# TruongKhang/cds-mvsnet

Hardware: AMD Instinct MI355X
Metric: depth-maps/sec per ref view at 640x512 N=5 D=192 (single-stage plane sweep incl. CostRegNet + regression) (higher is better)
Workload: dtype f32; 1 GPU; M1: single-stage StageNet volume 640x512, D=192, C=8, N=5 views; parallelism=single

## Files before the change

### cds_mvsnet_amd/csrc/cds_common.hpp

```cpp
#pragma once
#include <hip/hip_runtime.h>
#include <stdint.h>
#include <stdlib.h>

#include <atomic>

#include "../../include/cds_mvsnet_hip.h"

#define CDS_WAVE 64

#define CDS_ZMG_UNSUPPORTED 1
int cds_conv3d_zmg_dispatch(const float* x, const void* wsp, const float* bias, float* out, int Cin, int Cout, int D, int H, int W,
                            int stride, int pair, int act, hipStream_t st, const float* in_bound = nullptr, float w_inv = 1.f,
                            float* out_bound = nullptr);

using cds_f4 = float __attribute__((ext_vector_type(4)));

extern "C" int cds_debug_poison_lds(unsigned pattern);

static inline int cds_launch_status() {
  hipError_t e = hipGetLastError();
  if (const char* p = getenv("CDS_DEBUG_POISON_LDS")) {
    if (e == hipSuccess) (void)cds_debug_poison_lds((unsigned)strtoul(p, nullptr, 16));
  }
  return e == hipSuccess ? 0 : -(int)e;
}

static inline int cds_ceil_div(int a, int b) { return (a + b - 1) / b; }

static inline bool cds_env_is(const char* name, char c) { const char* e = getenv(name); return e && e[0] == c; }
static inline bool cds_env_set(const char* name) { return getenv(name) != nullptr; }
static inline int cds_env_int(const char* name, int dflt) { const char* e = getenv(name); return e ? atoi(e) : dflt; }

static inline int cds_allow_lds(const void* kernel, int bytes, std::atomic<unsigned long long>& mask) {
  int d = 0;
  (void)hipGetDevice(&d);
  const unsigned long long bit = 1ull << (d & 63);
  if (mask.load(std::memory_order_acquire) & bit) return 0;
  hipError_t e = hipFuncSetAttribute(kernel, hipFuncAttributeMaxDynamicSharedMemorySize, bytes);
  if (e != hipSuccess) { (void)hipGetLastError(); return -(int)e; }
  mask.fetch_or(bit, std::memory_order_release);
  return 0;
}

__device__ __forceinline__ int cds_xcd_remap(int bid, int nwg) {
  const int nx = 8;
  if (nwg < 2 * nx) return bid;
  int q = nwg / nx, r = nwg % nx;
  int xcd = bid % nx, idx = bid / nx;
  int base = xcd < r ? xcd * (q + 1) : r * (q + 1) + (xcd - r) * q;
  return base + idx;
}

__device__ __forceinline__ const float* cds_uniform_ptr(const float* p) {
  const uint64_t u = reinterpret_cast<uint64_t>(p);
  const uint32_t lo = __builtin_amdgcn_readfirstlane((uint32_t)u);
  const uint32_t hi = __builtin_amdgcn_readfirstlane((uint32_t)(u >> 32));
  return reinterpret_cast<const float*>(((uint64_t)hi << 32) | lo);
}

__device__ __forceinline__ float cds_act_conv(float v, int act) {
  if (act == CDS_ACT_RELU) return fmaxf(v, 0.0f);
  if (act == CDS_ACT_SIGMOID) return 1.0f / (1.0f + expf(-v));
  return v;
}

__device__ __forceinline__ float cds_apply_act(float v, int act) {
  switch (act) {
    case CDS_ACT_RELU: return fmaxf(v, 0.0f);
    case CDS_ACT_LEAKY01: return v > 0.0f ? v : v * 0.1f;
    case CDS_ACT_SIGMOID: return 1.0f / (1.0f + expf(-v));
    case CDS_ACT_TANH: return tanhf(v);
    default: return v;
  }
}
```

### cds_mvsnet_amd/csrc/conv3d_sbf.hip

```cpp
#include <stdlib.h>

#include "cds_common.hpp"
#include "sbf_common.hpp"

namespace {

#ifdef CDS_SBF_XFAST
#define SBF_TILE(tile, A, B, C) const int A = (tile) % tiles_x, B = ((tile) / tiles_x) % tiles_y, C = (tile) / (tiles_x * tiles_y)
#else
#define SBF_TILE(tile, A, B, C) \
  const int tiles_z_ = ntiles / (tiles_x * tiles_y); \
  const int C = (tile) % tiles_z_, A = ((tile) / tiles_z_) % tiles_x, B = (tile) / (tiles_z_ * tiles_x)
#endif

template <int S, int MB, int TX_, int TZ_, bool PAIR = false, bool WRES_ = false>
struct FCfg {
  static constexpr int TX = TX_, TY = 4, TZ = TZ_;
  static constexpr bool DEINT = S == 2 || PAIR;
  static constexpr int XT = TX / (PAIR ? 32 : 16), NT = XT * TZ;
  static constexpr int IX = (TX - 1) * S + 3, IY = (TY - 1) * S + 3, IZ = (TZ - 1) * S + 3;
  static constexpr int IXH = DEINT ? (IX + 1) / 2 : 0;
  static constexpr int IXP = DEINT ? 2 * IXH : (IX + 7) / 8 * 8;
  static constexpr int NPOS = IZ * IY * IXP;
  static constexpr int LDSB = NPOS * POSB;
// ... 698 lines not shown
      const unsigned char* tbuf = tiles + (st & 1) * Cfg::LDSB;
      const unsigned char* wr = wlds + rd * Tab::NKS * 3 * 1024;
      BV wa[2][3];
      BV bd[2][Cfg::NT][3];
      auto load_w = [&](int buf, int ks) {
        wa[buf][0].u = *reinterpret_cast<const uint4*>(wr + (ks * 3) * 1024);
        wa[buf][1].u = *reinterpret_cast<const uint4*>(wr + (ks * 3 + 1) * 1024);
        wa[buf][2].u = *reinterpret_cast<const uint4*>(wr + (ks * 3 + 2) * 1024);
      };
      auto load_b = [&](int buf, int ks) {
        const unsigned char* bp = tbuf + b_base + toff[ks];
#pragma unroll
        for (int q = 0; q < Cfg::NT; ++q) {
          const unsigned char* b = bp + q * 16 * POSB;
          bd[buf][q][0].u = *reinterpret_cast<const uint4*>(b);
          bd[buf][q][1].u = *reinterpret_cast<const uint4*>(b + 16);
          bd[buf][q][2].u = *reinterpret_cast<const uint4*>(b + 32);
        }
      };
      load_w(0, 0);
      load_b(0, 0);
#pragma unroll
      for (int ks = 0; ks < Tab::NKS; ++ks) {
        const int c = Tab::cls_of(ks), cur = ks & 1;
        if (ks + 1 < Tab::NKS) {
          load_b(cur ^ 1, ks + 1);
          load_w(cur ^ 1, ks + 1);
        }
        __builtin_amdgcn_sched_barrier(0);
        SBF_TERMS(acc[c], 0, Cfg::NT, wa[cur], bd[cur]);
      }
      if (rd + 1 == rounds && ay < H) {
#pragma unroll
        for (int c = 0; c < Tab::NCLS; ++c) {
          const size_t rowbase = ((size_t)(2 * az + (c >> 1)) * Ho + (2 * ay + (c & 1))) * Wo;
#pragma unroll
          for (int q = 0; q < Cfg::NT; ++q) {
            const int ax = tx_i * Cfg::CX + q * 16 + j;
            if (ax >= W) continue;
            const size_t base = (rowbase + 2 * ax + px) * Cout + co;
            const f32x4 a = acc[c][q];
            float4 o = make_float4(a.x + bv.x, a.y + bv.y, a.z + bv.z, a.w + bv.w);
            if (act == CDS_ACT_RELU) {
              o.x = fmaxf(o.x, 0.f); o.y = fmaxf(o.y, 0.f); o.z = fmaxf(o.z, 0.f); o.w = fmaxf(o.w, 0.f);
            }
            if (skip) {
              const float4 s4 = skv[c][q];
              o.x = s4.x + o.x; o.y = s4.y + o.y; o.z = s4.z + o.z; o.w = s4.w + o.w;
            }
            if (out_planar) {
              const size_t ovol = (size_t)(2 * D) * Ho * Wo;
              float* po = out + (size_t)co * ovol + (rowbase + 2 * ax + px);
#ifdef CDS_SBF_NTSTORE
              __builtin_nontemporal_store(o.x, po); __builtin_nontemporal_store(o.y, po + ovol);
              __builtin_nontemporal_store(o.z, po + 2 * ovol); __builtin_nontemporal_store(o.w, po + 3 * ovol);
#else
              po[0] = o.x; po[ovol] = o.y; po[2 * ovol] = o.z; po[3 * ovol] = o.w;
#endif
            } else {
              sbf_store4(out + base, o);
            }
          }
        }
      }
      __syncthreads();
    }
  }
}

template <int CYT>
int launch_deconv_ws_t(const float* x, const void* wsp, const float* b, const float* skip, float* out, int Cin, int Cout, int D, int H,
                       int W, int act, int out_planar, hipStream_t st) {
  using Cfg = DWSCfg<CYT>;
  const int tx = cds_ceil_div(W, Cfg::CX), ty = cds_ceil_div(H, Cfg::CY);
  const int ntiles = tx * ty * D;
  int tpw = max(1, min(16, ntiles / (256 * (CYT == 8 ? 1 : 2) * 8)));
  const int nwg = cds_ceil_div(ntiles, tpw);
  const int lds_bytes = (Cin >> 3) * DTab<true>::NKS * 3 * 1024 + 2 * Cfg::LDSB;
  static std::atomic<unsigned long long> lds_ok{0};
  if (int e_lds = cds_allow_lds(reinterpret_cast<const void*>(deconv3d_sbf_ws_kernel<CYT>), 160 * 1024, lds_ok)) return e_lds;
  hipLaunchKernelGGL(deconv3d_sbf_ws_kernel<CYT>, dim3(nwg), dim3(Cfg::THREADS), lds_bytes, st, x, reinterpret_cast<const uint4*>(wsp), b,
                     skip, out, Cin, Cout, D, H, W, act, out_planar, tx, ty, ntiles, tpw);
  return cds_launch_status();
}

int launch_deconv_ws(const float* x, const void* wsp, const float* b, const float* skip, float* out, int Cin, int Cout, int D, int H,
                     int W, int act, int out_planar, hipStream_t st) {
  const bool big = (H >= 16 && (long)cds_ceil_div(W, 32) * cds_ceil_div(H, 8) * D >= 2 * 256);
  if (big) return launch_deconv_ws_t<8>(x, wsp, b, skip, out, Cin, Cout, D, H, W, act, out_planar, st);
  return launch_deconv_ws_t<4>(x, wsp, b, skip, out, Cin, Cout, D, H, W, act, out_planar, st);
}

}

extern "C" int cds_conv3d_sbf_f32(const float* x, const void* weight_split, const float* bias, const float* skip, float* out,
                                  int Cin, int Cout, int D, int H, int W, int stride, int act, void* stream) {
  if (!x || !weight_split || !out || Cin < 8 || (Cin % 8) || Cout < 4 || (Cout % 4) || Cout > 64 || D < 1 || H < 1 || W < 1 ||
      (stride != 1 && stride != 2 && stride != CDS_SBF_PAIR))
    return CDS_EINVAL;
  if (stride == CDS_SBF_PAIR && Cout != 8) return CDS_EINVAL;
  hipStream_t st = (hipStream_t)stream;
  const int mb = (Cout + 15) / 16;
  if (!skip) {
    const int r = cds_conv3d_zmg_dispatch(x, weight_split, bias, out, Cin, Cout, D, H, W, stride == CDS_SBF_PAIR ? 1 : stride,
                                          stride == CDS_SBF_PAIR, act, st);
    if (r != CDS_ZMG_UNSUPPORTED) return r;
  }
  if (stride == CDS_SBF_PAIR) {
    if (Cout != 8) return CDS_EINVAL;
    if (Cin == 8) return launch_fwd<1, 1, 32, 4, true, true>(x, weight_split, bias, skip, out, Cin, Cout, D, H, W, act, st);
    return launch_fwd<1, 1, 32, 4, true>(x, weight_split, bias, skip, out, Cin, Cout, D, H, W, act, st);
  }
  if (stride == 1) {
    if (mb == 1) return launch_fwd<1, 1, 32, 4>(x, weight_split, bias, skip, out, Cin, Cout, D, H, W, act, st);
    if (mb == 2) return launch_fwd<1, 2, 32, 2>(x, weight_split, bias, skip, out, Cin, Cout, D, H, W, act, st);
    if (mb == 4) return launch_fwd<1, 4, 32, 2>(x, weight_split, bias, skip, out, Cin, Cout, D, H, W, act, st);
    return CDS_EINVAL;
  }
  if (mb == 1) return launch_fwd<2, 1, 16, 2>(x, weight_split, bias, skip, out, Cin, Cout, D, H, W, act, st);
  if (mb == 2) return launch_fwd<2, 2, 16, 2>(x, weight_split, bias, skip, out, Cin, Cout, D, H, W, act, st);
  if (mb == 4) return launch_fwd<2, 4, 16, 2>(x, weight_split, bias, skip, out, Cin, Cout, D, H, W, act, st);
  return CDS_EINVAL;
}

extern "C" int cds_conv3d_sf16_f32(const float* x, const void* weight_split, const float* bias, float* out, int Cin, int Cout, int D, int H,
                                   int W, int stride, int act, const float* in_bound, float w_inv_scale, float* out_bound, void* stream) {
  if (!x || !weight_split || !out || !in_bound || Cin < 8 || (Cin % 8) || Cout < 4 || (Cout % 4) || Cout > 64 || D < 1 || H < 1 || W < 1 ||
      (stride != 1 && stride != 2 && stride != CDS_SBF_PAIR) || !(w_inv_scale > 0.f))
    return CDS_EINVAL;
  if (stride == CDS_SBF_PAIR && Cout != 8) return CDS_EINVAL;
  hipStream_t st = (hipStream_t)stream;
  const int r = cds_conv3d_zmg_dispatch(x, weight_split, bias, out, Cin, Cout, D, H, W, stride == CDS_SBF_PAIR ? 1 : stride,
                                        stride == CDS_SBF_PAIR, act, st, in_bound, w_inv_scale, out_bound);
  if (r != CDS_ZMG_UNSUPPORTED) return r;
  const int mb = (Cout + 15) / 16;
  const int s_ = stride, Do = (D - 1) / s_ + 1, Ho = (H - 1) / s_ + 1, Wo = (W - 1) / s_ + 1;
  const long tiles = (long)cds_ceil_div(Wo, s_ == 1 ? 32 : 16) * cds_ceil_div(Ho, 4) * cds_ceil_div(Do, 2);
  const bool split = tiles <= cds_env_int("CDS_SBF_YSPLIT_TILES", 256) && !cds_env_is("CDS_SBF_YSPLIT", '0');
  if (split && stride == 1 && (mb == 2 || mb == 4))
    return launch_fwd<1, 1, 32, 2, false, false, true>(x, weight_split, bias, nullptr, out, Cin, Cout, D, H, W, act, st, in_bound, w_inv_scale, out_bound, mb);
  if (split && stride == 2 && mb == 4)
    return launch_fwd<2, 1, 16, 2, false, false, true>(x, weight_split, bias, nullptr, out, Cin, Cout, D, H, W, act, st, in_bound, w_inv_scale, out_bound, mb);
  if (stride == 1 && mb == 2) return launch_fwd<1, 2, 32, 2, false, false, true>(x, weight_split, bias, nullptr, out, Cin, Cout, D, H, W, act, st, in_bound, w_inv_scale, out_bound);
  if (stride == 1 && mb == 4) return launch_fwd<1, 4, 32, 2, false, false, true>(x, weight_split, bias, nullptr, out, Cin, Cout, D, H, W, act, st, in_bound, w_inv_scale, out_bound);
  if (stride == 2 && mb == 4) return launch_fwd<2, 4, 16, 2, false, false, true>(x, weight_split, bias, nullptr, out, Cin, Cout, D, H, W, act, st, in_bound, w_inv_scale, out_bound);
  return CDS_EINVAL;
}

extern "C" int cds_deconv3d_sf16_f32(const float* x, const void* weight_split, const float* bias, const float* skip, float* out, int Cin,
                                     int Cout, int D, int H, int W, int act, const float* in_bound, float w_inv_scale, float* out_bound,
                                     void* stream) {
  if (!x || !weight_split || !out || !in_bound || Cin < 8 || (Cin % 8) || Cout != 32 || D < 1 || H < 1 || W < 1 || !(w_inv_scale > 0.f))
    return CDS_EINVAL;
  const long tiles = (long)cds_ceil_div(W, 32) * cds_ceil_div(H, 4) * D;
  if (tiles <= cds_env_int("CDS_SBF_YSPLIT_TILES", 256) && !cds_env_is("CDS_SBF_YSPLIT", '0'))
    return launch_deconv<false, 1, true>(x, weight_split, bias, skip, out, Cin, Cout, D, H, W, act, 0, (hipStream_t)stream, in_bound,
                                         w_inv_scale, out_bound, 2);
  return launch_deconv<false, 2, true>(x, weight_split, bias, skip, out, Cin, Cout, D, H, W, act, 0, (hipStream_t)stream, in_bound,
                                       w_inv_scale, out_bound);
}

extern "C" int cds_deconv3d_sbf_f32(const float* x, const void* weight_split, const float* bias, const float* skip, float* out,
                                    int Cin, int Cout, int D, int H, int W, int act, int out_planar, void* stream) {
  if (!x || !weight_split || !out || Cin < 8 || (Cin % 8) || D < 1 || H < 1 || W < 1) return CDS_EINVAL;
  hipStream_t st = (hipStream_t)stream;
  if (Cout == 8) {
    if (Cin <= 32) return launch_deconv_ws(x, weight_split, bias, skip, out, Cin, Cout, D, H, W, act, out_planar, st);
    return launch_deconv<true, 1>(x, weight_split, bias, skip, out, Cin, Cout, D, H, W, act, out_planar, st);
  }
  if (Cout == 16) return launch_deconv<false, 1>(x, weight_split, bias, skip, out, Cin, Cout, D, H, W, act, out_planar, st);
  if (Cout == 32) return launch_deconv<false, 2>(x, weight_split, bias, skip, out, Cin, Cout, D, H, W, act, out_planar, st);
  return CDS_EINVAL;
}
```

### cds_mvsnet_amd/csrc/conv3d_zmg.hip

```cpp
#include <stdlib.h>

#include "cds_common.hpp"
#include "sbf_common.hpp"

namespace {

__device__ __attribute__((aligned(32))) float g_zmg_zeros[8];

template <int S_, int RD_, int MB_, bool PAIR_, int TXO_, int TYO_, int G_, int NG_, int CW_ = 4, bool F16_ = false, int RPW_ = 1,
          int YS_ = 1, int PF_ = 1>
struct ZG {
  static constexpr int S = S_, RD = RD_, MB = MB_, TXO = TXO_, TYO = TYO_, G = G_, NG = NG_;
  static constexpr bool F16 = F16_;
  static constexpr int NT = F16_ ? 2 : 3;
  static constexpr bool PAIR = PAIR_, DEINT = PAIR_ || S_ == 2;
  static constexpr int CW = CW_, PW = 4, THREADS = (CW + PW) * 64;
  static constexpr int RPW = RPW_, YS = YS_, PF = PF_;
  static_assert(PF == 1 || (PF == 2 && 2 * NG_ * (F16_ ? 2 : 3) <= 15), "operand prefetch distance (lgkmcnt is a 4-bit count)");
  static_assert(RD % RPW == 0 && MB % YS == 0, "rounds per wave / cout split");
  static constexpr int KSPL = RD / RPW, MBS = MB / YS;
  static_assert(CW % (KSPL * MBS) == 0 && (KSPL == 1 || KSPL == 2 || KSPL == 4), "consumer waves");
  static constexpr int PARTS = CW / (KSPL * MBS);
  static constexpr int ROWS = TYO / PARTS;
  static constexpr int XT = TXO / (PAIR ? 32 : 16);
// ... 213 lines not shown
      for (int jf = 0; jf < Cfg::NFIN; ++jf) {
        const int n = jf * 4 + k;
        if (n >= NTW) continue;
        const unsigned char* src = xch + (sp & 1) * Cfg::XCH1 + ((xgrp + n) * 4) * 1024 + lane * 16;
        f32x4 total = KEEP4 && k == 0 ? keep[jf] : *reinterpret_cast<const f32x4*>(src);
#pragma unroll
        for (int kk = 1; kk < 4; ++kk) total = total + (KEEP4 && kk == k ? keep[jf] : *reinterpret_cast<const f32x4*>(src + kk * 1024));
        store_tile_rt(n, sp, total);
      }
    } else {
#pragma unroll
      for (int n = 0; n < NTW; ++n) store_tile(n, sp, acc[n]);
    }
  };
  __syncthreads();
  for (int st = 0; st < nstages; ++st) {
    if (late && st > 0) finish(st - 1);
    int vpl[PAIR ? Cfg::NRES : 1];
    int vaddr[PAIR ? 1 : KS][PAIR ? 1 : G];
    {
      int sl[Cfg::NRES];
      int slot = (st * S * G) % R;
#pragma unroll
      for (int u = 0; u < Cfg::NRES; ++u) {
        sl[u] = slot * Cfg::PLANEB;
        slot = slot + 1 >= R ? slot + 1 - R : slot + 1;
      }
      if (PAIR) {
#pragma unroll
        for (int u = 0; u < Cfg::NRES; ++u) vpl[u] = lane_base + sl[u];
      } else {
#pragma unroll
        for (int t = 0; t < KS; ++t)
#pragma unroll
          for (int i = 0; i < G; ++i) {
            const int o0 = sl[S * i + Cfg::tap_kz(t, 0)] + Cfg::tap_off(t, 0), o1 = sl[S * i + Cfg::tap_kz(t, 1)] + Cfg::tap_off(t, 1);
            const int o2 = sl[S * i + Cfg::tap_kz(t, 2)] + Cfg::tap_off(t, 2), o3 = sl[S * i + Cfg::tap_kz(t, 3)] + Cfg::tap_off(t, 3);
            vaddr[t][i] = lane_base + (g == 0 ? o0 : (g == 1 ? o1 : (g == 2 ? o2 : o3)));
          }
      }
    }
    constexpr int NGRP = NTW / NG, NS = RPW * KS * NGRP;
    constexpr int PF = Cfg::PF;
    BV bd[PF + 1][NG][NT];
    auto load_b = [&](int buf, int ss) {
      const int t = (ss / NGRP) % KS, rr = ss / (NGRP * KS), grp = ss % NGRP;
#pragma unroll
      for (int q = 0; q < NG; ++q) {
        const int n = grp * NG + q, i = n % G, rx = n / G, xt = rx % Cfg::XT, r = rx / Cfg::XT;
        const unsigned char* b = lds + (PAIR ? vpl[PAIR ? S * i + t / 3 : 0] + (t % 3) * Cfg::IXP * POSB : vaddr[PAIR ? 0 : t][PAIR ? 0 : i]) +
                                 (r * S * Cfg::IXP + xt * 16) * POSB + rr * Cfg::SLICEB;
        bd[buf][q][0].u = *reinterpret_cast<const uint4*>(b);
        bd[buf][q][1].u = *reinterpret_cast<const uint4*>(b + 16);
        if (!F16) bd[buf][q][NT - 1].u = *reinterpret_cast<const uint4*>(b + 32);
      }
    };
    load_b(0, 0);
    if (PF == 2 && NS > 1) load_b(1, 1);
    __builtin_amdgcn_s_setprio(0);
#pragma unroll
    for (int t = 0; t < NTW; ++t) acc[t] = (f32x4){0.f, 0.f, 0.f, 0.f};
#pragma unroll
    for (int ss = 0; ss < NS; ++ss) {
      const int t = ss / NGRP, grp = ss % NGRP, db = ss % (PF + 1);
      if (ss + PF < NS) load_b((ss + PF) % (PF + 1), ss + PF);
      __builtin_amdgcn_sched_barrier(0);
#ifndef CDS_ZMG_LAZYWAIT
      if (ss + PF < NS) __builtin_amdgcn_s_waitcnt(0xC07F | ((PF * NT * NG) << 8));
      else if (PF == 2 && ss + 1 < NS) __builtin_amdgcn_s_waitcnt(0xC07F | ((NT * NG) << 8));
      else __builtin_amdgcn_s_waitcnt(0xC07F);
      __builtin_amdgcn_sched_barrier(0);
#endif
      if constexpr (F16) {
        SF16_TERMS(acc, grp * NG, NG, wres[t], bd[db]);
      } else {
        SBF_TERMS(acc, grp * NG, NG, wres[t], bd[db]);
      }
    }
    __builtin_amdgcn_s_setprio(CDS_ZMG_CPRIO);
    if (Cfg::KSPL == 2) {
      if (!late && st > 0) finish(st - 1);
      unsigned char* dst = xch + (st & 1) * Cfg::XCH1 + (wave * NH) * 1024 + lane * 16;
#pragma unroll
      for (int m = 0; m < NH; ++m) {
        *reinterpret_cast<f32x4*>(dst + m * 1024) = acc[(k ^ 1) * NH + m];
        keep[m] = acc[k * NH + m];
      }
    } else if (Cfg::KSPL == 4) {
      if (!late && st > 0) finish(st - 1);
      unsigned char* dst = xch + (st & 1) * Cfg::XCH1 + (xgrp * 4 + k) * 1024 + lane * 16;
#pragma unroll
      for (int n = 0; n < NTW; ++n) {
        if (KEEP4 && (n & 3) == k) keep[n >> 2] = acc[n];
        else *reinterpret_cast<f32x4*>(dst + n * 4096) = acc[n];
      }
    } else if (!late) {
      finish(st);
    }
    __syncthreads();
  }
  if (Cfg::KSPL >= 2 || late) finish(nstages - 1);
  if (F16) sf16_publish_bound(amax, out_bound);
}

inline int zmg_pick_nseg(int cols, int Do, int G) {
  const int nseg_env = cds_env_int("CDS_ZMG_NSEG", 0);
  if (nseg_env > 0) return nseg_env;
  const int stages = cds_ceil_div(Do, G);
  int best = 1;
  double best_cost = 1e30;
  for (int n = 1; n <= 32 && n <= stages; ++n) {
    const int per = cds_ceil_div(stages, n);
    if (n > 1 && per < 6) break;
    const double cost = (double)cds_ceil_div(cols * cds_ceil_div(stages, per), 256) * (per + 2.5);
    if (cost < best_cost - 1e-9) { best_cost = cost; best = n; }
  }
  return best;
}

template <class Cfg>
int launch_zmg(const float* x, const void* wsp, const float* b, float* out, int Cout, int D, int H, int W, int act, hipStream_t st,
               const float* in_bound = nullptr, float w_inv = 1.f, float* out_bound = nullptr, int min_wgs = 0) {
  constexpr int S = Cfg::S;
  const int Do = (D - 1) / S + 1, Ho = (H - 1) / S + 1, Wo = (W - 1) / S + 1;
  const int tx = cds_ceil_div(Wo, Cfg::TXO), ty = cds_ceil_div(Ho, Cfg::TYO);
  int nseg = zmg_pick_nseg(tx * ty * Cfg::YS, Do, Cfg::G);
  const int zseg = cds_ceil_div(cds_ceil_div(Do, nseg), Cfg::G) * Cfg::G;
  nseg = cds_ceil_div(Do, zseg);
  if (min_wgs > 0 && tx * ty * nseg * Cfg::YS < min_wgs) return CDS_ZMG_UNSUPPORTED;
  auto kern = conv3d_zmg_kernel<Cfg>;
  static std::atomic<unsigned long long> lds_ok{0};
  if (int e_lds = cds_allow_lds(reinterpret_cast<const void*>(kern), Cfg::LDSB, lds_ok)) return e_lds;
  hipLaunchKernelGGL(kern, dim3(tx * ty * nseg, Cfg::YS), dim3(Cfg::THREADS), Cfg::LDSB, st, x, reinterpret_cast<const uint4*>(wsp), b,
                     out, Cout, D, H, W, Do, Ho, Wo, act, tx, ty, zseg, in_bound, w_inv, out_bound);
  return cds_launch_status();
}

}

int cds_conv3d_zmg_dispatch(const float* x, const void* wsp, const float* bias, float* out, int Cin, int Cout, int D, int H, int W,
                            int stride, int pair, int act, hipStream_t st, const float* in_bound, float w_inv, float* out_bound) {
  if (in_bound) {
    if (pair) {
      if (Cin == 8) return launch_zmg<ZG<1, 1, 1, true, 32, 8, 3, 1, 8, true>>(x, wsp, bias, out, Cout, D, H, W, act, st, in_bound, w_inv, out_bound);
      if (Cin == 16) return launch_zmg<ZG<1, 2, 1, true, 32, 8, 1, 4, 4, true>>(x, wsp, bias, out, Cout, D, H, W, act, st, in_bound, w_inv, out_bound);
      if (Cin == 32) return launch_zmg<ZG<1, 4, 1, true, 32, 3, 1, 3, 4, true>>(x, wsp, bias, out, Cout, D, H, W, act, st, in_bound, w_inv, out_bound);
      return CDS_ZMG_UNSUPPORTED;
    }
    if (stride == 1 && Cin == 16 && Cout == 16)
      return launch_zmg<ZG<1, 2, 1, false, 32, 8, 1, 1, 8, true>>(x, wsp, bias, out, Cout, D, H, W, act, st, in_bound, w_inv, out_bound);
    if (stride == 2 && Cin == 8 && Cout == 16)
      return launch_zmg<ZG<2, 1, 1, false, 16, 8, 1, 1, 8, true>>(x, wsp, bias, out, Cout, D, H, W, act, st, in_bound, w_inv, out_bound);
    if (stride == 2 && Cin == 16 && Cout == 32)
      return launch_zmg<ZG<2, 2, 2, false, 16, 4, 1, 1, 8, true>>(x, wsp, bias, out, Cout, D, H, W, act, st, in_bound, w_inv, out_bound);
    const int deep = cds_env_is("CDS_ZMG", '0') ? 0 : cds_env_int("CDS_ZMG_DEEP", 1);
    const int min_wgs = deep == 2 ? 0 : 256;
    if (deep > 0 && stride == 1 && Cin == 32 && Cout == 32)
      return launch_zmg<ZG<1, 4, 2, false, 16, 4, 1, 1, 8, true, 1, 1, 2>>(x, wsp, bias, out, Cout, D, H, W, act, st, in_bound, w_inv, out_bound, min_wgs);
    if (deep > 0 && stride == 1 && Cin == 64 && Cout == 64)
      return launch_zmg<ZG<1, 8, 4, false, 16, 2, 1, 1, 8, true, 2, 2>>(x, wsp, bias, out, Cout, D, H, W, act, st, in_bound, w_inv, out_bound, min_wgs);
    return CDS_ZMG_UNSUPPORTED;
  }
  const bool off = cds_env_is("CDS_ZMG", '0');
  if (off) return CDS_ZMG_UNSUPPORTED;
  if (pair) {
    if (Cin == 8) return launch_zmg<ZG<1, 1, 1, true, 32, 8, 3, 1, 8>>(x, wsp, bias, out, Cout, D, H, W, act, st);
    if (Cin == 16) return launch_zmg<ZG<1, 2, 1, true, 32, 8, 1, 4>>(x, wsp, bias, out, Cout, D, H, W, act, st);
    if (Cin == 32) return launch_zmg<ZG<1, 4, 1, true, 32, 3, 1, 3>>(x, wsp, bias, out, Cout, D, H, W, act, st);
    return CDS_ZMG_UNSUPPORTED;
  }
  if (stride == 1) {
    if (Cin == 16 && Cout == 16) return launch_zmg<ZG<1, 2, 1, false, 32, 8, 1, 1, 8>>(x, wsp, bias, out, Cout, D, H, W, act, st);
    return CDS_ZMG_UNSUPPORTED;
  }
  if (Cin == 8 && Cout == 16) return launch_zmg<ZG<2, 1, 1, false, 16, 8, 1, 1, 8>>(x, wsp, bias, out, Cout, D, H, W, act, st);
  if (Cin == 16 && Cout == 32) return launch_zmg<ZG<2, 2, 2, false, 16, 4, 1, 1, 8>>(x, wsp, bias, out, Cout, D, H, W, act, st);
  return CDS_ZMG_UNSUPPORTED;
}
```

### cds_mvsnet_amd/csrc/deconv3d_zm.hip

```cpp
#include "sbf_common.hpp"

namespace {

template <int ROUNDS_>
struct DZC {
  static constexpr int ROUNDS = ROUNDS_;
  static constexpr int TX = 16, TY = 8;
  static constexpr int IX = TX + 1, IY = TY + 1, IXP = 18;
  static constexpr int ROUNDB = IY * IXP * POSB;
  static constexpr int SLOTB = ROUNDS * ROUNDB;
  static constexpr int NSLOT = 3;
  static constexpr int CW = 8, PW = 4, THREADS = (CW + PW) * 64;
  static constexpr int LDS = NSLOT * SLOTB;
  static constexpr int NITEM = IY * IX * ROUNDS;
  static constexpr int IPT = (NITEM + PW * 64 - 1) / (PW * 64);
};

template <int ROUNDS, bool F16>
__global__ __launch_bounds__((DZC<ROUNDS>::THREADS), 3) void deconv3d_zm_kernel(
    const float* __restrict__ x, const uint4* __restrict__ wcls, const float* __restrict__ bias, const float* __restrict__ skip,
    float* __restrict__ out, int D, int H, int W, int tiles_x, int ncols, int seg_len, int act, const float* __restrict__ in_bound,
    float w_inv, float* __restrict__ out_bound) {
  using C = DZC<ROUNDS>;
  constexpr int NT = F16 ? 2 : 3;
  const float xs = F16 ? sf16_scale(in_bound[0]) : 1.0f;
  const float out_mul = F16 ? w_inv / xs : 1.0f;
  constexpr int Cin = 8 * ROUNDS, Cout = 16;
  extern __shared__ __attribute__((aligned(16))) unsigned char lds[];
  const int tid = threadIdx.x;
  const int lane = tid & 63;
  const int wave = __builtin_amdgcn_readfirstlane(tid >> 6);
  const int wg = cds_xcd_remap(blockIdx.x, gridDim.x);
  const int col = wg % ncols, seg = wg / ncols;
  const int tx_i = col % tiles_x, ty_i = col / tiles_x;
  const int a0 = seg * seg_len, a1 = min(D, a0 + seg_len);
  if (a0 >= a1) return;
  const int X0 = tx_i * C::TX, Y0 = ty_i * C::TY;
  const int Ho = 2 * H, Wo = 2 * W;

  if (wave >= C::CW) {
    __builtin_amdgcn_s_setprio(3);
    const int ptid = tid - C::CW * 64;
    int s_src[C::IPT], s_dst[C::IPT];
#pragma unroll
    for (int h = 0; h < C::IPT; ++h) {
      const int it = h * C::PW * 64 + ptid;
      const int rd = it % ROUNDS, p = it / ROUNDS;
      const int row = p / C::IX, c = p - row * C::IX;
      const int gy = Y0 + row, gx = X0 + c;
      const bool ok = it < C::NITEM && gy < H && gx < W;
      s_src[h] = ok ? ((gy * W + gx) * Cin + rd * 8) : -1;
      s_dst[h] = it < C::NITEM ? rd * C::ROUNDB + (row * C::IXP + c) * POSB : -1;
    }
    float4 va[C::IPT], vb[C::IPT];
    auto issue = [&](int plane) {
      const bool pok = plane < D;
      const float* __restrict__ xp = x + (size_t)min(plane, D - 1) * H * W * Cin;
#pragma unroll
      for (int h = 0; h < C::IPT; ++h) {
        const bool ok = pok && s_src[h] >= 0;
        const float* src = xp + (ok ? s_src[h] : 0);
        const float4 a = *reinterpret_cast<const float4*>(src), b = *reinterpret_cast<const float4*>(src + 4);
        va[h] = ok ? a : make_float4(0.f, 0.f, 0.f, 0.f);
        vb[h] = ok ? b : make_float4(0.f, 0.f, 0.f, 0.f);
      }
    };
    auto deposit = [&](int plane) {
      unsigned char* base = lds + (plane % C::NSLOT) * C::SLOTB;
#pragma unroll
      for (int h = 0; h < C::IPT; ++h)
        if (s_dst[h] >= 0) {
          if (F16) split_store8_f16(base + s_dst[h], va[h], vb[h], xs);
          else split_store8(base + s_dst[h], va[h], vb[h]);
        }
    };
    issue(a0);
    deposit(a0);
    issue(a0 + 1);
    deposit(a0 + 1);
    issue(a0 + 2);
    __syncthreads();
    for (int a = a0; a < a1; ++a) {
      deposit(a + 2);
      issue(a + 3);
      __syncthreads();
    }
    return;
  }

  const int pz = wave >> 2, py = (wave >> 1) & 1, px = wave & 1;
  if (pz) __builtin_amdgcn_s_setprio(1);
  const int j = lane & 15, g = lane >> 4;
  BV wlo[ROUNDS][3], whi[ROUNDS][3];
  {
    const uint4* __restrict__ wp = wcls + (size_t)wave * ROUNDS * 2 * 3 * 64 + lane;
#pragma unroll
    for (int rd = 0; rd < ROUNDS; ++rd)
#pragma unroll
      for (int k = 0; k < NT; ++k) {
        wlo[rd][k].u = wp[((rd * 2 + 0) * 3 + k) * 64];
        whi[rd][k].u = wp[((rd * 2 + 1) * 3 + k) * 64];
      }
  }
  const float4 bv = bias ? *reinterpret_cast<const float4*>(bias + 4 * g) : make_float4(0.f, 0.f, 0.f, 0.f);
  const int b_off = (((g >> 1) * C::IXP) + j + (g & 1)) * POSB;
  const int xv = 2 * (X0 + j) + px;
  const bool x_ok = X0 + j < W;
  const size_t zstride = (size_t)Ho * Wo * Cout;
  float amax = 0.f;
  __syncthreads();
  for (int a = a0; a < a1; ++a) {
    const unsigned char* lo = lds + (a % C::NSLOT) * C::SLOTB + b_off;
    const unsigned char* hi = lds + ((a + 1) % C::NSLOT) * C::SLOTB + b_off;
    const size_t zbase = (size_t)(2 * a + pz) * zstride;
    const int nrows = min(C::TY, H - Y0);
    float4 skn = make_float4(0.f, 0.f, 0.f, 0.f);
    auto row_off = [&](int n) { return ((size_t)(2 * (Y0 + n) + py) * Wo + xv) * Cout + 4 * g; };
    if (skip && x_ok) skn = *reinterpret_cast<const float4*>(skip + zbase + row_off(0));
    asm volatile("" ::"v"(skn.x), "v"(skn.y), "v"(skn.z), "v"(skn.w));
    for (int n = 0; n < nrows; ++n) {
      const float4 sk = skn;
      if (skip && x_ok && n + 1 < nrows) skn = *reinterpret_cast<const float4*>(skip + zbase + row_off(n + 1));
      f32x4 acc[1] = {F16 ? (f32x4){0.f, 0.f, 0.f, 0.f} : (f32x4){bv.x, bv.y, bv.z, bv.w}};
      const unsigned char* lo_n = lo + n * C::IXP * POSB;
      const unsigned char* hi_n = hi + n * C::IXP * POSB;
#pragma unroll
      for (int rd = 0; rd < ROUNDS; ++rd) {
        BV b[1][3];
        b[0][0].u = *reinterpret_cast<const uint4*>(lo_n + rd * C::ROUNDB);
        b[0][1].u = *reinterpret_cast<const uint4*>(lo_n + rd * C::ROUNDB + 16);
        if constexpr (F16) {
          SF16_TERMS(acc, 0, 1, wlo[rd], b);
        } else {
          b[0][2].u = *reinterpret_cast<const uint4*>(lo_n + rd * C::ROUNDB + 32);
          SBF_TERMS(acc, 0, 1, wlo[rd], b);
        }
        if (pz) {
          BV c[1][3];
          c[0][0].u = *reinterpret_cast<const uint4*>(hi_n + rd * C::ROUNDB);
          c[0][1].u = *reinterpret_cast<const uint4*>(hi_n + rd * C::ROUNDB + 16);
          if constexpr (F16) {
            SF16_TERMS(acc, 0, 1, whi[rd], c);
          } else {
            c[0][2].u = *reinterpret_cast<const uint4*>(hi_n + rd * C::ROUNDB + 32);
            SBF_TERMS(acc, 0, 1, whi[rd], c);
          }
        }
      }
      asm volatile("" ::"v"(skn.x), "v"(skn.y), "v"(skn.z), "v"(skn.w));
      if (x_ok) {
        const f32x4 r = acc[0];
        float4 o = F16 ? make_float4(r.x * out_mul + bv.x, r.y * out_mul + bv.y, r.z * out_mul + bv.z, r.w * out_mul + bv.w)
                       : make_float4(r.x, r.y, r.z, r.w);
        if (act == CDS_ACT_RELU) o = make_float4(fmaxf(o.x, 0.f), fmaxf(o.y, 0.f), fmaxf(o.z, 0.f), fmaxf(o.w, 0.f));
        if (skip) o = make_float4(sk.x + o.x, sk.y + o.y, sk.z + o.z, sk.w + o.w);
        if (F16) amax = fmaxf(fmaxf(amax, fmaxf(fabsf(o.x), fabsf(o.y))), fmaxf(fabsf(o.z), fabsf(o.w)));
        sbf_store4(out + zbase + row_off(n), o);
      }
    }
    __syncthreads();
  }
  if (F16) sf16_publish_bound(amax, out_bound);
}

}

static int dzm_entry(const float* x, const void* weight_cls, const float* bias, const float* skip, float* out, int Cin, int Cout, int D,
                     int H, int W, int act, const float* in_bound, float w_inv, float* out_bound, void* stream) {
  if (!x || !weight_cls || !out || Cin != 32 || Cout != 16 || D < 1 || H < 1 || W < 1) return CDS_EINVAL;
  if ((long)2 * H * 2 * W * Cout >= (1l << 31) || (long)H * W * Cin >= (1l << 31)) return CDS_EINVAL;
  using C = DZC<4>;
  hipStream_t st = (hipStream_t)stream;
  const int tiles_x = cds_ceil_div(W, C::TX), tiles_y = cds_ceil_div(H, C::TY);
  const int ncols = tiles_x * tiles_y;
  const char* nseg_e = getenv("CDS_DZM_NSEG");
  int best = 1;
  double best_cost = 1e30;
  for (int n = 1; n <= min(D, 24); ++n) {
    const int len = cds_ceil_div(D, n);
    const int n_eff = cds_ceil_div(D, len);
    const double cost = (double)cds_ceil_div(ncols * n_eff, 256) * (len + 1.5);
    if (cost < best_cost - 1e-9) { best_cost = cost; best = n; }
  }
  if (nseg_e && atoi(nseg_e) > 0) best = min(atoi(nseg_e), D);
  const int seg_len = cds_ceil_div(D, best);
  const int nseg = cds_ceil_div(D, seg_len);
  if (in_bound) {
    static std::atomic<unsigned long long> lds_ok_h{0};
    if (int e_lds = cds_allow_lds(reinterpret_cast<const void*>(deconv3d_zm_kernel<4, true>), 160 * 1024, lds_ok_h)) return e_lds;
    hipLaunchKernelGGL((deconv3d_zm_kernel<4, true>), dim3(ncols * nseg), dim3(C::THREADS), C::LDS, st, x,
                       reinterpret_cast<const uint4*>(weight_cls), bias, skip, out, D, H, W, tiles_x, ncols, seg_len, act, in_bound, w_inv,
                       out_bound);
    return cds_launch_status();
  }
  static std::atomic<unsigned long long> lds_ok{0};
  if (int e_lds = cds_allow_lds(reinterpret_cast<const void*>(deconv3d_zm_kernel<4, false>), 160 * 1024, lds_ok)) return e_lds;
  hipLaunchKernelGGL((deconv3d_zm_kernel<4, false>), dim3(ncols * nseg), dim3(C::THREADS), C::LDS, st, x,
                     reinterpret_cast<const uint4*>(weight_cls), bias, skip, out, D, H, W, tiles_x, ncols, seg_len, act, nullptr, 1.0f,
                     nullptr);
  return cds_launch_status();
}

extern "C" int cds_deconv3d_zm_f32(const float* x, const void* weight_cls, const float* bias, const float* skip, float* out,
                                   int Cin, int Cout, int D, int H, int W, int act, void* stream) {
  return dzm_entry(x, weight_cls, bias, skip, out, Cin, Cout, D, H, W, act, nullptr, 1.0f, nullptr, stream);
}

extern "C" int cds_deconv3d_zm_sf16_f32(const float* x, const void* weight_cls, const float* bias, const float* skip, float* out,
                                        int Cin, int Cout, int D, int H, int W, int act, const float* in_bound, float w_inv_scale,
                                        float* out_bound, void* stream) {
  if (!in_bound || !(w_inv_scale > 0.f)) return CDS_EINVAL;
  return dzm_entry(x, weight_cls, bias, skip, out, Cin, Cout, D, H, W, act, in_bound, w_inv_scale, out_bound, stream);
}
```

Baseline: 182.6 depth-maps/s.

## Add warp-specialized zm64 deconv kernel for Cin=64 Cout=32 sf16 path

Adds a new producer/consumer deconv kernel for the Cin=64, Cout=32 scaled-f16 transposed conv, and routes it in ahead of the generic split deconv. The kernel uses 4-row tiles, splits the output channels into two grid.y blocks, and keeps per-wave weights in registers, spilling part of the second tap set to LDS. The input producer is factored into a shared helper, and one zmg stride-2 config gets an extra template argument. This adds register and LDS pressure, and the numerics of the new kernel are unverified.

```diff
diff --git a/cds_mvsnet_amd/csrc/cds_common.hpp b/cds_mvsnet_amd/csrc/cds_common.hpp
--- a/cds_mvsnet_amd/csrc/cds_common.hpp
+++ b/cds_mvsnet_amd/csrc/cds_common.hpp
@@ -13,6 +13,8 @@
 int cds_conv3d_zmg_dispatch(const float* x, const void* wsp, const float* bias, float* out, int Cin, int Cout, int D, int H, int W,
                             int stride, int pair, int act, hipStream_t st, const float* in_bound = nullptr, float w_inv = 1.f,
                             float* out_bound = nullptr);
+int cds_deconv3d_zm64_dispatch(const float* x, const void* wsp, const float* bias, const float* skip, float* out, int Cin, int Cout,
+                               int D, int H, int W, int act, hipStream_t st, const float* in_bound, float w_inv, float* out_bound);
 
 using cds_f4 = float __attribute__((ext_vector_type(4)));
 
diff --git a/cds_mvsnet_amd/csrc/conv3d_sbf.hip b/cds_mvsnet_amd/csrc/conv3d_sbf.hip
--- a/cds_mvsnet_amd/csrc/conv3d_sbf.hip
+++ b/cds_mvsnet_amd/csrc/conv3d_sbf.hip
@@ -874,6 +874,11 @@
                                      void* stream) {
   if (!x || !weight_split || !out || !in_bound || Cin < 8 || (Cin % 8) || Cout != 32 || D < 1 || H < 1 || W < 1 || !(w_inv_scale > 0.f))
     return CDS_EINVAL;
+  {
+    const int r = cds_deconv3d_zm64_dispatch(x, weight_split, bias, skip, out, Cin, Cout, D, H, W, act, (hipStream_t)stream, in_bound,
+                                             w_inv_scale, out_bound);
+    if (r != CDS_ZMG_UNSUPPORTED) return r;
+  }
   const long tiles = (long)cds_ceil_div(W, 32) * cds_ceil_div(H, 4) * D;
   if (tiles <= cds_env_int("CDS_SBF_YSPLIT_TILES", 256) && !cds_env_is("CDS_SBF_YSPLIT", '0'))
     return launch_deconv<false, 1, true>(x, weight_split, bias, skip, out, Cin, Cout, D, H, W, act, 0, (hipStream_t)stream, in_bound,
diff --git a/cds_mvsnet_amd/csrc/conv3d_zmg.hip b/cds_mvsnet_amd/csrc/conv3d_zmg.hip
--- a/cds_mvsnet_amd/csrc/conv3d_zmg.hip
+++ b/cds_mvsnet_amd/csrc/conv3d_zmg.hip
@@ -389,7 +389,7 @@
     if (stride == 2 && Cin == 8 && Cout == 16)
       return launch_zmg<ZG<2, 1, 1, false, 16, 8, 1, 1, 8, true>>(x, wsp, bias, out, Cout, D, H, W, act, st, in_bound, w_inv, out_bound);
     if (stride == 2 && Cin == 16 && Cout == 32)
-      return launch_zmg<ZG<2, 2, 2, false, 16, 4, 1, 1, 8, true>>(x, wsp, bias, out, Cout, D, H, W, act, st, in_bound, w_inv, out_bound);
+      return launch_zmg<ZG<2, 2, 2, false, 16, 4, 1, 1, 8, true, 2>>(x, wsp, bias, out, Cout, D, H, W, act, st, in_bound, w_inv, out_bound);
     const int deep = cds_env_is("CDS_ZMG", '0') ? 0 : cds_env_int("CDS_ZMG_DEEP", 1);
     const int min_wgs = deep == 2 ? 0 : 256;
     if (deep > 0 && stride == 1 && Cin == 32 && Cout == 32)
diff --git a/cds_mvsnet_amd/csrc/deconv3d_zm.hip b/cds_mvsnet_amd/csrc/deconv3d_zm.hip
--- a/cds_mvsnet_amd/csrc/deconv3d_zm.hip
+++ b/cds_mvsnet_amd/csrc/deconv3d_zm.hip
@@ -2,10 +2,10 @@
 
 namespace {
 
-template <int ROUNDS_>
+template <int ROUNDS_, int TY_ = 8>
 struct DZC {
   static constexpr int ROUNDS = ROUNDS_;
-  static constexpr int TX = 16, TY = 8;
+  static constexpr int TX = 16, TY = TY_;
   static constexpr int IX = TX + 1, IY = TY + 1, IXP = 18;
   static constexpr int ROUNDB = IY * IXP * POSB;
   static constexpr int SLOTB = ROUNDS * ROUNDB;
@@ -16,6 +16,57 @@
   static constexpr int IPT = (NITEM + PW * 64 - 1) / (PW * 64);
 };
 
+template <class C, bool F16>
+__device__ __forceinline__ void dzm_produce(const float* __restrict__ x, unsigned char* lds, int ptid, int X0, int Y0, int D, int H, int W,
+                                            int a0, int a1, float xs) {
+  constexpr int ROUNDS = C::ROUNDS, Cin = 8 * ROUNDS;
+  __builtin_amdgcn_s_setprio(3);
+  int s_src[C::IPT], s_dst[C::IPT];
+#pragma unroll
+  for (int h = 0; h < C::IPT; ++h) {
+    const int it = h * C::PW * 64 + ptid;
+    const int rd = it % ROUNDS, p = it / ROUNDS;
+    const int row = p / C::IX, c = p - row * C::IX;
+    const int gy = Y0 + row, gx = X0 + c;
+    const bool ok = it < C::NITEM && gy < H && gx < W;
+    s_src[h] = ok ? ((gy * W + gx) * Cin + rd * 8) : -1;
+    s_dst[h] = it < C::NITEM ? rd * C::ROUNDB + (row * C::IXP + c) * POSB : -1;
+  }
+  float4 va[C::IPT], vb[C::IPT];
+  auto issue = [&](int plane) {
+    const bool pok = plane < D;
+    const float* __restrict__ xp = x + (size_t)min(plane, D - 1) * H * W * Cin;
+#pragma unroll
+    for (int h = 0; h < C::IPT; ++h) {
+      const bool ok = pok && s_src[h] >= 0;
+      const float* src = xp + (ok ? s_src[h] : 0);
+      const float4 a = *reinterpret_cast<const float4*>(src), b = *reinterpret_cast<const float4*>(src + 4);
+      va[h] = ok ? a : make_float4(0.f, 0.f, 0.f, 0.f);
+      vb[h] = ok ? b : make_float4(0.f, 0.f, 0.f, 0.f);
+    }
+  };
+  auto deposit = [&](int plane) {
+    unsigned char* base = lds + (plane % C::NSLOT) * C::SLOTB;
+#pragma unroll
+    for (int h = 0; h < C::IPT; ++h)
+      if (s_dst[h] >= 0) {
+        if (F16) split_store8_f16(base + s_dst[h], va[h], vb[h], xs);
+        else split_store8(base + s_dst[h], va[h], vb[h]);
+      }
+  };
+  issue(a0);
+  deposit(a0);
+  issue(a0 + 1);
+  deposit(a0 + 1);
+  issue(a0 + 2);
+  __syncthreads();
+  for (int a = a0; a < a1; ++a) {
+    deposit(a + 2);
+    issue(a + 3);
+    __syncthreads();
+  }
+}
+
 template <int ROUNDS, bool F16>
 __global__ __launch_bounds__((DZC<ROUNDS>::THREADS), 3) void deconv3d_zm_kernel(
     const float* __restrict__ x, const uint4* __restrict__ wcls, const float* __restrict__ bias, const float* __restrict__ skip,
@@ -25,7 +76,7 @@
   constexpr int NT = F16 ? 2 : 3;
   const float xs = F16 ? sf16_scale(in_bound[0]) : 1.0f;
   const float out_mul = F16 ? w_inv / xs : 1.0f;
-  constexpr int Cin = 8 * ROUNDS, Cout = 16;
+  constexpr int Cout = 16;
   extern __shared__ __attribute__((aligned(16))) unsigned char lds[];
   const int tid = threadIdx.x;
   const int lane = tid & 63;
@@ -39,52 +90,7 @@
   const int Ho = 2 * H, Wo = 2 * W;
 
   if (wave >= C::CW) {
-    __builtin_amdgcn_s_setprio(3);
-    const int ptid = tid - C::CW * 64;
-    int s_src[C::IPT], s_dst[C::IPT];
-#pragma unroll
-    for (int h = 0; h < C::IPT; ++h) {
-      const int it = h * C::PW * 64 + ptid;
-      const int rd = it % ROUNDS, p = it / ROUNDS;
-      const int row = p / C::IX, c = p - row * C::IX;
-      const int gy = Y0 + row, gx = X0 + c;
-      const bool ok = it < C::NITEM && gy < H && gx < W;
-      s_src[h] = ok ? ((gy * W + gx) * Cin + rd * 8) : -1;
-      s_dst[h] = it < C::NITEM ? rd * C::ROUNDB + (row * C::IXP + c) * POSB : -1;
-    }
-    float4 va[C::IPT], vb[C::IPT];
-    auto issue = [&](int plane) {
-      const bool pok = plane < D;
-      const float* __restrict__ xp = x + (size_t)min(plane, D - 1) * H * W * Cin;
-#pragma unroll
-      for (int h = 0; h < C::IPT; ++h) {
-        const bool ok = pok && s_src[h] >= 0;
-        const float* src = xp + (ok ? s_src[h] : 0);
-        const float4 a = *reinterpret_cast<const float4*>(src), b = *reinterpret_cast<const float4*>(src + 4);
-        va[h] = ok ? a : make_float4(0.f, 0.f, 0.f, 0.f);
-        vb[h] = ok ? b : make_float4(0.f, 0.f, 0.f, 0.f);
-      }
-    };
-    auto deposit = [&](int plane) {
-      unsigned char* base = lds + (plane % C::NSLOT) * C::SLOTB;
-#pragma unroll
-      for (int h = 0; h < C::IPT; ++h)
-        if (s_dst[h] >= 0) {
-          if (F16) split_store8_f16(base + s_dst[h], va[h], vb[h], xs);
-          else split_store8(base + s_dst[h], va[h], vb[h]);
-        }
-    };
-    issue(a0);
-    deposit(a0);
-    issue(a0 + 1);
-    deposit(a0 + 1);
-    issue(a0 + 2);
-    __syncthreads();
-    for (int a = a0; a < a1; ++a) {
-      deposit(a + 2);
-      issue(a + 3);
-      __syncthreads();
-    }
+    dzm_produce<C, F16>(x, lds, tid - C::CW * 64, X0, Y0, D, H, W, a0, a1, xs);
     return;
   }
 
@@ -163,6 +169,144 @@
   if (F16) sf16_publish_bound(amax, out_bound);
 }
 
+
+constexpr int DZM64_W1L = 2;
+__global__ __launch_bounds__((DZC<8, 4>::THREADS), 3) void deconv3d_zm64_kernel(
+    const float* __restrict__ x, const uint4* __restrict__ wsp, const float* __restrict__ bias, const float* __restrict__ skip,
+    float* __restrict__ out, int D, int H, int W, int tiles_x, int ncols, int seg_len, int act, const float* __restrict__ in_bound,
+    float w_inv, float* __restrict__ out_bound) {
+  using C = DZC<8, 4>;
+  constexpr int ROUNDS = 8, Cout = 32, NKS = 9, W1L = DZM64_W1L;
+  const float xs = sf16_scale(in_bound[0]);
+  const float out_mul = w_inv / xs;
+  extern __shared__ __attribute__((aligned(16))) unsigned char lds[];
+  const int tid = threadIdx.x;
+  const int lane = tid & 63;
+  const int wave = __builtin_amdgcn_readfirstlane(tid >> 6);
+  const int wg = cds_xcd_remap(blockIdx.x, gridDim.x);
+  const int mbtot = gridDim.y, mb0 = blockIdx.y;
+  const int col = wg % ncols, seg = wg / ncols;
+  const int tx_i = col % tiles_x, ty_i = col / tiles_x;
+  const int a0 = seg * seg_len, a1 = min(D, a0 + seg_len);
+  if (a0 >= a1) return;
+  const int X0 = tx_i * C::TX, Y0 = ty_i * C::TY;
+  const int Ho = 2 * H, Wo = 2 * W;
+
+  if (wave >= C::CW) {
+    dzm_produce<C, true>(x, lds, tid - C::CW * 64, X0, Y0, D, H, W, a0, a1, xs);
+    return;
+  }
+
+  const int pz = wave >> 2, py = (wave >> 1) & 1, px = wave & 1;
+  const bool two = wave == 7;
+  if (two) __builtin_amdgcn_s_setprio(1);
+  const int j = lane & 15, g = lane >> 4;
+  BV w0[ROUNDS][2], w1[ROUNDS - W1L][2];
+  unsigned char* w1l = lds + C::LDS + lane * 16;
+  {
+    const uint4* __restrict__ wp = wsp + lane;
+#pragma unroll
+    for (int rd = 0; rd < ROUNDS; ++rd)
+#pragma unroll
+      for (int k = 0; k < 2; ++k) {
+        w0[rd][k].u = wp[(size_t)(((rd * NKS + wave) * mbtot + mb0) * 3 + k) * 64];
+        const uint4 v = wp[(size_t)(((rd * NKS + (two ? 8 : wave)) * mbtot + mb0) * 3 + k) * 64];
+        if (rd < ROUNDS - W1L) w1[rd][k].u = v;
+        else if (two) *reinterpret_cast<uint4*>(w1l + ((rd - (ROUNDS - W1L)) * 2 + k) * 1024) = v;
+      }
+  }
+  const float4 bv = bias ? *reinterpret_cast<const float4*>(bias + mb0 * 16 + 4 * g) : make_float4(0.f, 0.f, 0.f, 0.f);
+  const int ny = 1 + py, nx = 1 + px;
+  const bool live = g < (1 + pz) * ny * nx;
+  const int dz = live ? g / (ny * nx) : 0, dy = live ? (g / nx) % ny : 0, dx = live ? g % nx : 0;
+  const int b_off = ((dy * C::IXP) + j + dx) * POSB;
+  const int xv = 2 * (X0 + j) + px;
+  const bool x_ok = X0 + j < W;
+  const size_t zstride = (size_t)Ho * Wo * Cout;
+  const int nrows = min(C::TY, H - Y0);
+  float amax = 0.f;
+  __syncthreads();
+  for (int a = a0; a < a1; ++a) {
+    const unsigned char* p0 = lds + (a % C::NSLOT) * C::SLOTB + b_off;
+    const unsigned char* hi = lds + ((a + 1) % C::NSLOT) * C::SLOTB + b_off;
+    const unsigned char* lo = dz ? hi : p0;
+    const size_t zbase = (size_t)(2 * a + pz) * zstride;
+    float4 skn = make_float4(0.f, 0.f, 0.f, 0.f);
+    auto row_off = [&](int n) { return ((size_t)(2 * (Y0 + n) + py) * Wo + xv) * Cout + mb0 * 16 + 4 * g; };
+    if (skip && x_ok) skn = *reinterpret_cast<const float4*>(skip + zbase + row_off(0));
+    asm volatile("" ::"v"(skn.x), "v"(skn.y), "v"(skn.z), "v"(skn.w));
+    for (int n = 0; n < nrows; ++n) {
+      const float4 sk = skn;
+      if (skip && x_ok && n + 1 < nrows) skn = *reinterpret_cast<const float4*>(skip + zbase + row_off(n + 1));
+      f32x4 acc[1] = {(f32x4){0.f, 0.f, 0.f, 0.f}};
+      const unsigned char* lo_n = lo + n * C::IXP * POSB;
+      const unsigned char* hi_n = hi + n * C::IXP * POSB;
+#pragma unroll
+      for (int rd = 0; rd < ROUNDS; ++rd) {
+        BV b[1][2];
+        b[0][0].u = *reinterpret_cast<const uint4*>(lo_n + rd * C::ROUNDB);
+        b[0][1].u = *reinterpret_cast<const uint4*>(lo_n + rd * C::ROUNDB + 16);
+        SF16_TERMS(acc, 0, 1, w0[rd], b);
+        if (two) {
+          BV c[1][2];
+          c[0][0].u = *reinterpret_cast<const uint4*>(hi_n + rd * C::ROUNDB);
+          c[0][1].u = *reinterpret_cast<const uint4*>(hi_n + rd * C::ROUNDB + 16);
+          if (rd < ROUNDS - W1L) {
+            SF16_TERMS(acc, 0, 1, w1[rd < ROUNDS - W1L ? rd : 0], c);
+          } else {
+            BV wl[2];
+            wl[0].u = *reinterpret_cast<const uint4*>(w1l + ((rd - (ROUNDS - W1L)) * 2 + 0) * 1024);
+            wl[1].u = *reinterpret_cast<const uint4*>(w1l + ((rd - (ROUNDS - W1L)) * 2 + 1) * 1024);
+            SF16_TERMS(acc, 0, 1, wl, c);
+          }
+        }
+      }
+      asm volatile("" ::"v"(skn.x), "v"(skn.y), "v"(skn.z), "v"(skn.w));
+      if (x_ok) {
+        const f32x4 r = acc[0];
+        float4 o = make_float4(r.x * out_mul + bv.x, r.y * out_mul + bv.y, r.z * out_mul + bv.z, r.w * out_mul + bv.w);
+        if (act == CDS_ACT_RELU) o = make_float4(fmaxf(o.x, 0.f), fmaxf(o.y, 0.f), fmaxf(o.z, 0.f), fmaxf(o.w, 0.f));
+        if (skip) o = make_float4(sk.x + o.x, sk.y + o.y, sk.z + o.z, sk.w + o.w);
+        amax = fmaxf(fmaxf(amax, fmaxf(fabsf(o.x), fabsf(o.y))), fmaxf(fabsf(o.z), fabsf(o.w)));
+        sbf_store4(out + zbase + row_off(n), o);
+      }
+    }
+    __syncthreads();
+  }
+  sf16_publish_bound(amax, out_bound);
+}
+
+int dzm_pick_nseg(int wgs_per_seg, int D) {
+  int best = 1;
+  double best_cost = 1e30;
+  for (int n = 1; n <= min(D, 24); ++n) {
+    const int len = cds_ceil_div(D, n);
+    const int n_eff = cds_ceil_div(D, len);
+    const double cost = (double)cds_ceil_div(wgs_per_seg * n_eff, 256) * (len + 1.5);
+    if (cost < best_cost - 1e-9) { best_cost = cost; best = n; }
+  }
+  const int nseg_e = cds_env_int("CDS_DZM_NSEG", 0);
+  return nseg_e > 0 ? min(nseg_e, D) : best;
+}
+
+}
+
+int cds_deconv3d_zm64_dispatch(const float* x, const void* wsp, const float* bias, const float* skip, float* out, int Cin, int Cout,
+                               int D, int H, int W, int act, hipStream_t st, const float* in_bound, float w_inv, float* out_bound) {
+  const int deep = cds_env_int("CDS_DZM_DEEP", 1);
+  if (deep <= 0 || Cin != 64 || Cout != 32 || !in_bound) return CDS_ZMG_UNSUPPORTED;
+  if ((long)2 * H * 2 * W * Cout >= (1l << 31) || (long)H * W * Cin >= (1l << 31)) return CDS_ZMG_UNSUPPORTED;
+  using C = DZC<8, 4>;
+  const int tiles_x = cds_ceil_div(W, C::TX), tiles_y = cds_ceil_div(H, C::TY);
+  const int ncols = tiles_x * tiles_y;
+  const int seg_len = cds_ceil_div(D, dzm_pick_nseg(ncols * 2, D));
+  const int nseg = cds_ceil_div(D, seg_len);
+  if (deep == 1 && ncols * nseg * 2 < 256) return CDS_ZMG_UNSUPPORTED;
+  static std::atomic<unsigned long long> lds_ok{0};
+  if (int e_lds = cds_allow_lds(reinterpret_cast<const void*>(deconv3d_zm64_kernel), 160 * 1024, lds_ok)) return e_lds;
+  hipLaunchKernelGGL(deconv3d_zm64_kernel, dim3(ncols * nseg, 2), dim3(C::THREADS), C::LDS + DZM64_W1L * 2 * 1024, st, x, reinterpret_cast<const uint4*>(wsp),
+                     bias, skip, out, D, H, W, tiles_x, ncols, seg_len, act, in_bound, w_inv, out_bound);
+  return cds_launch_status();
 }
 
 static int dzm_entry(const float* x, const void* weight_cls, const float* bias, const float* skip, float* out, int Cin, int Cout, int D,
@@ -173,17 +317,7 @@
   hipStream_t st = (hipStream_t)stream;
   const int tiles_x = cds_ceil_div(W, C::TX), tiles_y = cds_ceil_div(H, C::TY);
   const int ncols = tiles_x * tiles_y;
-  const char* nseg_e = getenv("CDS_DZM_NSEG");
-  int best = 1;
-  double best_cost = 1e30;
-  for (int n = 1; n <= min(D, 24); ++n) {
-    const int len = cds_ceil_div(D, n);
-    const int n_eff = cds_ceil_div(D, len);
-    const double cost = (double)cds_ceil_div(ncols * n_eff, 256) * (len + 1.5);
-    if (cost < best_cost - 1e-9) { best_cost = cost; best = n; }
-  }
-  if (nseg_e && atoi(nseg_e) > 0) best = min(atoi(nseg_e), D);
-  const int seg_len = cds_ceil_div(D, best);
+  const int seg_len = cds_ceil_div(D, dzm_pick_nseg(ncols, D));
   const int nseg = cds_ceil_div(D, seg_len);
   if (in_bound) {
     static std::atomic<unsigned long long> lds_ok_h{0};
```

After: 186.0 depth-maps/s, median of 6. 1.02x the previous value.
